# jinlinyi/PerspectiveFields

Hardware: NVIDIA H100
Metric: images/sec at 640x480 (Paramnet-360Cities-edina), H100 vs ref CPU (higher is better)
Workload: dtype f32 via 3x bf16 split MMA, fp32 accumulate

## Files before the change

### include/pf_b200.h

```cpp
#ifndef PF_B200_H_
#define PF_B200_H_

#include <stddef.h>
#include <stdint.h>

#ifdef __cplusplus
extern "C" {
#endif

#define PF_ABI_VERSION 3

typedef struct pf_engine* pf_handle;

enum pf_status { PF_OK = 0, PF_ERR_ARG = -1, PF_ERR_CUDA = -2, PF_ERR_WEIGHT = -3, PF_ERR_WORKSPACE = -4 };

enum pf_dtype { PF_F32 = 0, PF_BF16 = 1 };

enum pf_param_net { PF_PARAM_NONE = 0, PF_PARAM_CENTERED = 1 , PF_PARAM_UNCENTERED = 2  };

typedef struct pf_model_desc {
  int gravity_classes;
  int latitude_classes;
  int param_net;
  int param_input_size;
// ... 189 lines not shown
  int phase4;
  int npred; pf_tma_pred pred[2];
  int force_bn, force_kb;
  int picked_bn, picked_kb;
  int force_sched, picked_sched;
} pf_tma_op;
int pf_op_tma(pf_tma_op* op, void* stream);
int pf_op_tma_bf16(pf_tma_op* op, void* stream);
int pf_op_conv1_ring(const void* c_hi, const void* c_lo, int B, int H, int W, const float* wf, const float* bias, float* out,
                     const float* pg_w, const float* pg_b, float* pg_out, const float* pl_w, const float* pl_b, float* pl_out, void* stream);
int pf_tma_pick_tile(int mode, int64_t M, int N, int K, int sm_count, int* bn, int* kb);
int pf_op_pn_wgrad(const float* dy, int ldy, const float* x, const void* x_hi, const void* x_lo, int op, int ldx, int64_t R, int N, int K,
                   float* out, int* S, int* chunk, void* stream);
int pf_op_pn_colsum(const float* src, int64_t R, int C, float* out, void* stream);
int pf_op_pn_ln_bwd(const float* x, const float* dy, int64_t R, int C, const float* w, float* dx, float* g, void* stream);
int pf_op_pn_dw7_bwd(const float* x, const float* dt, int B, int H, int W, int C, const float* w_rot, float* dw, float* dx, int* rows_per_block,
                     void* stream);
int pf_op_pn_stem_bwd(const float* pin, const float* dS, const float* w, int B, int OH, int OW, float* dw, float* dpin, int* rows_per_block,
                      void* stream);
int pf_op_pn_fields_grad(const float* dpin, int B, int IH, int IW, int OH, int OW, float* dgrav, float* dlat, void* stream);
int pf_op_pn_tail_bwd(const float* feat, int n, int HW, const float* nw, const float* nb, const float* hw, const float* draw, float* dx,
                      float* grads, void* stream);
int pf_op_pn_pw2_grads(const float* G, const float* sdy, int C, int K, const float* gamma, const void* w_hi, const void* w_lo, const float* b,
                       float* dW, float* db, float* dgamma, void* stream);
int pf_op_pn_gelu_bwd(const float* dh, float* u, int64_t n, void* hi, void* lo, void* stream);
int pf_op_pn_scale_split(const float* src, const float* scale, int64_t n, int C, void* hi, void* lo, void* stream);
int pf_op_pn_col2im2(const float* dP, int B, int H, int W, int C, float* out, void* stream);
int pf_op_layernorm(const float* x, float* y, int64_t rows, int C, const float* w, const float* b, float eps, void* stream);
int pf_op_attention_tc(const float* q, const float* kv, float* out, int B, int N, int C, int heads, void* stream);
int pf_op_attention_tc_bf16(const float* q, const float* kv, float* out, int B, int N, int C, int heads, void* stream);
int pf_op_attention_tc_keys(const float* q, const float* kv, float* out, int B, int N, int NKV, int C, int heads, int bf16, void* stream);
int pf_op_dwconv3x3_gelu(const float* x, float* y, int B, int H, int W, int C, const float* w9c, const float* bias, void* stream);
int pf_op_dwconv7x7(const float* x, float* y, int B, int H, int W, int C, const float* w49c, const float* bias, void* stream);
int pf_op_upsample2x(const float* x, float* y, int B, int H, int W, int C, void* stream);
int pf_op_preprocess(const uint8_t* img_dev, int H, int W, const float* mean3, const float* std3, float* y, void* stream);
int pf_op_preprocess_sized(const uint8_t* img_dev, int H, int W, int net_h, int net_w, const float* mean3, const float* std3, float* y, void* stream);
int pf_op_resize_u8(const uint8_t* img_dev, int H, int W, int new_h, int new_w, uint8_t* out_dev, void* stream);
int pf_op_resize_f32(const float* img_dev, int H, int W, int C, int new_h, int new_w, float* out_dev, void* stream);
int pf_op_fill_stream(float* dst, int64_t numel, float value, void* stream);
int pf_op_argmax_decode(const float* logits, float* field, int B, int HW, int NC, int is_gravity, void* stream);
int pf_op_pred_argmax_decode(const float* feat, int ld, int coff, const float* w, const float* bias, float* field, int B, int HW, int NC,
                             int is_gravity, void* stream);
int pf_op_postprocess(const float* vec, const float* lat, int n, const int32_t* height, const int32_t* width,
                      float* gravity_original, const int64_t* gravity_original_offset, float* latitude_original,
                      const int64_t* latitude_original_offset, int lat_is_sin, void* stream);
int pf_op_postprocess_sized(const float* vec, const float* lat, int n, int net_h, int net_w, const int32_t* height, const int32_t* width,
                            float* gravity_original, const int64_t* gravity_original_offset, float* latitude_original,
                            const int64_t* latitude_original_offset, int lat_is_sin, void* stream);

#ifdef __cplusplus
}
#endif
#endif
```

### perspectivefields_b200/_native.py

```python
import ctypes
import os
import subprocess

_HERE = os.path.dirname(os.path.abspath(__file__))
ROOT = os.path.dirname(_HERE)
LIB_PATH = os.path.join(_HERE, "libpf_b200.so")
SRC_DIR = os.path.join(_HERE, "csrc")
HEADER = os.path.join(ROOT, "include", "pf_b200.h")

PF_F32, PF_BF16 = 0, 1
PF_PARAM_NONE, PF_PARAM_CENTERED, PF_PARAM_UNCENTERED = 0, 1, 2

NVCC_FLAGS = ["-gencode", "arch=compute_90a,code=sm_90a", "-O3", "-lineinfo", "-std=c++17",
              "-Xcompiler", "-fPIC", "-shared", "-ldl"]


class pf_model_desc(ctypes.Structure):
    _fields_ = [("gravity_classes", ctypes.c_int), ("latitude_classes", ctypes.c_int), ("param_net", ctypes.c_int),
                ("param_input_size", ctypes.c_int), ("pixel_mean", ctypes.c_float * 3), ("pixel_std", ctypes.c_float * 3)]


class pf_camera(ctypes.Structure):
    _fields_ = [("height", ctypes.c_int32), ("width", ctypes.c_int32), ("focal_rel", ctypes.c_double), ("elevation", ctypes.c_double),
                ("roll", ctypes.c_double), ("cx_rel", ctypes.c_double), ("cy_rel", ctypes.c_double),
# ... 149 lines not shown
        "pf_camera_fields": (i32, [i32, ctypes.POINTER(pf_camera), i32, vp, vp, vp]),
        "pf_camera_fields_vp": (i32, [i32, ctypes.POINTER(pf_camera), ctypes.POINTER(ctypes.c_double), i32, vp, vp, vp]),
        "pf_draw_fields": (i32, [i32, ctypes.POINTER(pf_draw_canvas), i32, vp, vp, vp, vp, vp]),
        "pf_pano_views": (i32, [i32, vp, i32, i32, ctypes.POINTER(pf_pano_view), i32, vp, vp, vp, vp, vp, vp, vp, vp, vp]),
        "pf_equi_views": (i32, [i32, vp, i32, i32, i32, i32, ctypes.POINTER(pf_equi_view), i32, i32, i32, i32, vp, vp]),
        "pf_encode_fields": (i32, [i32, i32, i32, i32, vp, ctypes.POINTER(i64), vp, ctypes.POINTER(i64), i32, i32, i32, vp, vp, vp]),
        "pf_head_losses_workspace": (i64, [i32, i32, i32, i32, i32]),
        "pf_head_losses": (i32, [i32, i32, i32, i32, i32, vp, vp, i32, vp, vp, i32, i32, f32, f32, vp, vp, i64, vp]),
        "pf_field_errors_workspace": (i64, [ctypes.POINTER(pf_field_image), i32, i32]),
        "pf_field_errors": (i32, [i32, ctypes.POINTER(pf_field_image), i32, vp, vp, vp, vp, vp, i32, ctypes.POINTER(ctypes.c_double), i32,
                                  vp, vp, vp, vp, vp, vp, vp, i64, vp]),
        "pf_fit_camera_workspace": (i64, [ctypes.POINTER(pf_fit_image), i32]),
        "pf_fit_camera": (i32, [i32, ctypes.POINTER(pf_fit_image), i32, vp, vp, vp, i32, ctypes.c_double, i32, vp, vp, vp, vp, vp, i64, vp]),
        "pf_rectify_workspace": (i64, [ctypes.POINTER(pf_rectify_image), i32]),
        "pf_rectify_views": (i32, [i32, ctypes.POINTER(pf_rectify_image), i32, vp, vp, vp, vp, i32, vp, i32, i32, ctypes.c_double, i32,
                                   ctypes.POINTER(ctypes.c_int32), vp, vp, vp, i64, vp]),
        "pf_op_pn_wgrad": (i32, [vp, i32, vp, vp, vp, i32, i32, i64, i32, i32, vp, ctypes.POINTER(i32), ctypes.POINTER(i32), vp]),
        "pf_op_pn_colsum": (i32, [vp, i64, i32, vp, vp]),
        "pf_op_pn_ln_bwd": (i32, [vp, vp, i64, i32, vp, vp, vp, vp]),
        "pf_op_pn_dw7_bwd": (i32, [vp, vp, i32, i32, i32, i32, vp, vp, vp, ctypes.POINTER(i32), vp]),
        "pf_op_pn_stem_bwd": (i32, [vp, vp, vp, i32, i32, i32, vp, vp, ctypes.POINTER(i32), vp]),
        "pf_op_pn_fields_grad": (i32, [vp, i32, i32, i32, i32, i32, vp, vp, vp]),
        "pf_op_pn_tail_bwd": (i32, [vp, i32, i32, vp, vp, vp, vp, vp, vp, vp]),
        "pf_op_pn_pw2_grads": (i32, [vp, vp, i32, i32, vp, vp, vp, vp, vp, vp, vp, vp]),
        "pf_op_pn_gelu_bwd": (i32, [vp, vp, i64, vp, vp, vp]),
        "pf_op_pn_scale_split": (i32, [vp, vp, i64, i32, vp, vp, vp]),
        "pf_op_pn_col2im2": (i32, [vp, i32, i32, i32, i32, vp, vp]),
        "pf_op_layernorm": (i32, [vp, vp, i64, i32, vp, vp, f32, vp]),
        "pf_op_attention_tc": (i32, [vp, vp, vp, i32, i32, i32, i32, vp]),
        "pf_op_attention_tc_bf16": (i32, [vp, vp, vp, i32, i32, i32, i32, vp]),
        "pf_op_attention_tc_keys": (i32, [vp, vp, vp, i32, i32, i32, i32, i32, i32, vp]),
        "pf_op_dwconv3x3_gelu": (i32, [vp, vp, i32, i32, i32, i32, vp, vp, vp]),
        "pf_op_dwconv7x7": (i32, [vp, vp, i32, i32, i32, i32, vp, vp, vp]),
        "pf_op_upsample2x": (i32, [vp, vp, i32, i32, i32, i32, vp]),
        "pf_op_preprocess": (i32, [vp, i32, i32, ctypes.POINTER(f32), ctypes.POINTER(f32), vp, vp]),
        "pf_op_preprocess_sized": (i32, [vp, i32, i32, i32, i32, ctypes.POINTER(f32), ctypes.POINTER(f32), vp, vp]),
        "pf_op_resize_u8": (i32, [vp, i32, i32, i32, i32, vp, vp]),
        "pf_op_resize_f32": (i32, [vp, i32, i32, i32, i32, i32, vp, vp]),
        "pf_op_argmax_decode": (i32, [vp, vp, i32, i32, i32, i32, vp]),
        "pf_op_fill_stream": (i32, [vp, i64, f32, vp]),
        "pf_op_pred_argmax_decode": (i32, [vp, i32, i32, vp, vp, vp, i32, i32, i32, i32, vp]),
        "pf_op_postprocess": (i32, [vp, vp, i32, ctypes.POINTER(ctypes.c_int32), ctypes.POINTER(ctypes.c_int32), vp, ctypes.POINTER(i64), vp,
                                    ctypes.POINTER(i64), i32, vp]),
        "pf_op_postprocess_sized": (i32, [vp, vp, i32, i32, i32, ctypes.POINTER(ctypes.c_int32), ctypes.POINTER(ctypes.c_int32), vp,
                                          ctypes.POINTER(i64), vp, ctypes.POINTER(i64), i32, vp]),
        "pf_comm_unique_id": (i32, [vp]),
        "pf_comm_create": (i32, [i32, i32, i32, vp, ctypes.POINTER(vp)]),
        "pf_comm_destroy": (i32, [vp]),
        "pf_gather": (i32, [vp, i32, i32, ctypes.POINTER(vp), ctypes.POINTER(i64), ctypes.POINTER(ctypes.c_int32), vp]),
        "pf_jpeg_create": (i32, [i32, i32, ctypes.POINTER(vp)]),
        "pf_jpeg_destroy": (i32, [vp]),
        "pf_jpeg_info": (i32, [vp, vp, i64, ctypes.POINTER(ctypes.c_int32), ctypes.POINTER(ctypes.c_int32)]),
        "pf_jpeg_decode_batch": (i32, [vp, i32, ctypes.POINTER(vp), ctypes.POINTER(i64), ctypes.POINTER(ctypes.c_int32),
                                       ctypes.POINTER(ctypes.c_int32), vp, ctypes.POINTER(i64), vp]),
    }
    for name, (res, args) in sig.items():
        try:
            fn = getattr(L, name)
        except AttributeError:
            if os.environ.get("PF_B200_LIB"):
                continue
            raise
        fn.restype, fn.argtypes = res, args
    if L.pf_abi_version() != 3:
        raise RuntimeError("libpf_b200.so ABI version mismatch")
    _lib = L
    return L


EXPORTS = ["pf_abi_version", "pf_last_error", "pf_kernel_launch_count", "pf_create", "pf_create_sized", "pf_destroy", "pf_set_weight",
           "pf_finalize", "pf_workspace_bytes", "pf_forward", "pf_param_workspace_bytes", "pf_param_forward", "pf_param_train_workspace_bytes",
           "pf_param_train_forward", "pf_param_backward", "pf_param_grad_numel", "pf_param_grad_entry", "pf_profile_enable", "pf_profile_read", "pf_profile_kernels_enable",
           "pf_profile_kernels_read", "pf_set_option", "pf_debug_enable", "pf_debug_count", "pf_debug_name", "pf_debug_numel",
           "pf_debug_copy", "pf_camera_fields", "pf_camera_fields_vp", "pf_pano_views", "pf_equi_views", "pf_draw_fields",
           "pf_encode_fields", "pf_head_losses_workspace", "pf_head_losses", "pf_field_errors_workspace", "pf_field_errors",
           "pf_fit_camera_workspace", "pf_fit_camera", "pf_rectify_workspace", "pf_rectify_views", "pf_comm_unique_id", "pf_comm_create", "pf_comm_destroy", "pf_gather",
           "pf_jpeg_create", "pf_jpeg_destroy", "pf_jpeg_info", "pf_jpeg_decode_batch",
           "pf_op_conv_gemm", "pf_op_tma", "pf_op_tma_bf16", "pf_op_conv1_ring", "pf_tma_pick_tile", "pf_op_layernorm",
           "pf_op_attention_tc", "pf_op_attention_tc_bf16", "pf_op_attention_tc_keys", "pf_op_dwconv3x3_gelu",
           "pf_op_dwconv7x7", "pf_op_upsample2x", "pf_op_preprocess", "pf_op_preprocess_sized", "pf_op_fill_stream", "pf_op_resize_u8",
           "pf_op_resize_f32", "pf_op_argmax_decode", "pf_op_pred_argmax_decode", "pf_op_postprocess", "pf_op_postprocess_sized",
           "pf_op_pn_wgrad", "pf_op_pn_colsum", "pf_op_pn_ln_bwd", "pf_op_pn_dw7_bwd", "pf_op_pn_stem_bwd", "pf_op_pn_fields_grad",
           "pf_op_pn_tail_bwd", "pf_op_pn_pw2_grads", "pf_op_pn_gelu_bwd", "pf_op_pn_scale_split", "pf_op_pn_col2im2"]


class PfError(RuntimeError):
    pass


def check(status):
    if status < 0:
        raise PfError(f"libpf_b200: {lib().pf_last_error().decode()} (status {status})")
    return status
```

### perspectivefields_b200/csrc/layers.cuh

```cuda
#pragma once
#include "common.cuh"

namespace pf {

template <int KH, int KW, int STRIDE, int PAD, int COUT, int PPT, int PGROUPS>
__global__ void __launch_bounds__(COUT* PGROUPS) stem_conv_kernel(const float* __restrict__ in, int ldin, int B, int H, int W,
                                                                  const float* __restrict__ w, const float* __restrict__ bias,
                                                                  float* __restrict__ out, int OH, int OW) {
  constexpr int PIX = PPT * PGROUPS;
  constexpr int IN_W = (PIX - 1) * STRIDE + KW;
  __shared__ float s_in[KH][IN_W][3];
  const int tiles_x = cdiv(OW, PIX);
  int bid = blockIdx.x;
  const int tx = bid % tiles_x; bid /= tiles_x;
  const int oy = bid % OH; const int b = bid / OH;
  const int ox0 = tx * PIX;
  const int iy0 = oy * STRIDE - PAD, ix0 = ox0 * STRIDE - PAD;
  for (int i = threadIdx.x; i < KH * IN_W * 3; i += blockDim.x) {
    const int c = i % 3, x = (i / 3) % IN_W, y = i / (3 * IN_W);
    const int iy = iy0 + y, ix = ix0 + x;
    float v = 0.f;
    if ((unsigned)iy < (unsigned)H && (unsigned)ix < (unsigned)W) v = __ldg(in + ((long long)(b * H + iy) * W + ix) * ldin + c);
    s_in[y][x][c] = v;
  }
// ... 219 lines not shown
            acc[oy][p].z = fmaf(a[p + kx].z, kk.z, acc[oy][p].z); acc[oy][p].w = fmaf(a[p + kx].w, kk.w, acc[oy][p].w);
          }
        }
      }
    }
#endif
#pragma unroll
    for (int oy = 0; oy < 2; ++oy) {
      if (y0 + oy >= H) break;
#pragma unroll
      for (int p = 0; p < PX; ++p) {
        if (!cv[p + 1]) break;
        const float4 o = make_float4(gelu_erf(acc[oy][p].x), gelu_erf(acc[oy][p].y), gelu_erf(acc[oy][p].z), gelu_erf(acc[oy][p].w));
        const unsigned oi = o00 + (unsigned)oy * rs + (unsigned)p * C4;
        if (out) reinterpret_cast<float4*>(out)[oi] = o;
        if (shi) {
          uint2 h, l;
          split_bf16x2(o.x, o.y, h.x, l.x);
          split_bf16x2(o.z, o.w, h.y, l.y);
          reinterpret_cast<uint2*>(shi)[oi] = h;
          reinterpret_cast<uint2*>(slo)[oi] = l;
        }
      }
    }
  }
}

#ifndef PF_DW7_PX
#define PF_DW7_PX 4
#endif
#ifndef PF_DW7_MINBLOCKS
#define PF_DW7_MINBLOCKS 2
#endif
__global__ void __launch_bounds__(256, PF_DW7_MINBLOCKS) dwconv7x7_kernel(const float* __restrict__ in, float* __restrict__ out, int B, int H, int W, int C,
                                                        const float* __restrict__ w, const float* __restrict__ bias) {
  pdl_wait();
  pdl_launch();
  constexpr int PX = PF_DW7_PX;
  const unsigned C4 = (unsigned)C >> 2, XG = ((unsigned)W + PX - 1) / PX, YG = ((unsigned)H + 1) >> 1;
  const unsigned total = (unsigned)B * YG * XG * C4;
  const unsigned rs = (unsigned)W * C4;
  const float4* __restrict__ in4 = reinterpret_cast<const float4*>(in);
  const float4* __restrict__ w4 = reinterpret_cast<const float4*>(w);
  for (unsigned i = blockIdx.x * blockDim.x + threadIdx.x; i < total; i += gridDim.x * blockDim.x) {
    const unsigned c4 = i % C4;
    unsigned r = i / C4;
    const unsigned xg = r % XG; r /= XG;
    const int y0 = (int)(r % YG) * 2; const unsigned b = r / YG;
    const int x0 = (int)xg * PX;
    const unsigned o00 = ((b * (unsigned)H + (unsigned)y0) * (unsigned)W + (unsigned)x0) * C4 + c4;
    bool cv[PX + 6];
#pragma unroll
    for (int j = 0; j < PX + 6; ++j) cv[j] = (unsigned)(x0 - 3 + j) < (unsigned)W;
    const float4 bv = __ldg(reinterpret_cast<const float4*>(bias) + c4);
    float4 acc[2][PX];
#pragma unroll
    for (int oy = 0; oy < 2; ++oy)
#pragma unroll
      for (int p = 0; p < PX; ++p) acc[oy][p] = bv;
#pragma unroll
    for (int ry = 0; ry < 8; ++ry) {
      const int iy = y0 + ry - 3;
      if ((unsigned)iy >= (unsigned)H) continue;
      const unsigned rb = o00 + (unsigned)(ry - 3) * rs - 3u * C4;
      float4 a[PX + 6];
#pragma unroll
      for (int j = 0; j < PX + 6; ++j) {
        a[j] = make_float4(0.f, 0.f, 0.f, 0.f);
        if (cv[j]) a[j] = __ldg(in4 + (rb + (unsigned)j * C4));
      }
#pragma unroll
      for (int oy = 0; oy < 2; ++oy) {
        const int ky = ry - oy;
        if (ky < 0 || ky > 6) continue;
#pragma unroll
        for (int kx = 0; kx < 7; ++kx) {
          const float4 k = __ldg(w4 + ((unsigned)(ky * 7 + kx) * C4 + c4));
#pragma unroll
          for (int p = 0; p < PX; ++p) {
            acc[oy][p].x = fmaf(a[p + kx].x, k.x, acc[oy][p].x); acc[oy][p].y = fmaf(a[p + kx].y, k.y, acc[oy][p].y);
            acc[oy][p].z = fmaf(a[p + kx].z, k.z, acc[oy][p].z); acc[oy][p].w = fmaf(a[p + kx].w, k.w, acc[oy][p].w);
          }
        }
      }
    }
#pragma unroll
    for (int oy = 0; oy < 2; ++oy) {
      if (y0 + oy >= H) break;
#pragma unroll
      for (int p = 0; p < PX; ++p) {
        if (!cv[p + 3]) break;
        reinterpret_cast<float4*>(out)[o00 + (unsigned)oy * rs + (unsigned)p * C4] = acc[oy][p];
      }
    }
  }
}

inline unsigned ew_grid(long long total) {
  long long g = cdivl(total, 256);
  const long long cap = 132LL * 32;
  return (unsigned)(g < cap ? (g > 0 ? g : 1) : cap);
}

inline long long upsample2x_threads(int B, int H, int W, int C) { return (long long)B * H * ((W + 1) / 2) * (C / 4); }
__global__ void __launch_bounds__(256) upsample2x_kernel(const float* __restrict__ in, int ldi, int icoff, float* __restrict__ out, int ldo, int ocoff,
                                                         int B, int H, int W, int C, __nv_bfloat16* __restrict__ shi = nullptr, __nv_bfloat16* __restrict__ slo = nullptr) {
  pdl_wait();
  pdl_launch();
  const unsigned C4 = (unsigned)C >> 2, JG = ((unsigned)W + 1) >> 1, li4 = (unsigned)ldi >> 2, lo4 = (unsigned)ldo >> 2;
  const unsigned total = (unsigned)B * H * JG * C4;
  const unsigned OW = 2u * W;
  const float4* __restrict__ in4 = reinterpret_cast<const float4*>(in + icoff);
  const unsigned oc4 = (unsigned)ocoff >> 2;
  for (unsigned i = blockIdx.x * blockDim.x + threadIdx.x; i < total; i += gridDim.x * blockDim.x) {
    const unsigned c4 = i % C4;
    unsigned r = i / C4;
    const unsigned jg = r % JG; r /= JG;
    const int iy = (int)(r % (unsigned)H); const unsigned b = r / (unsigned)H;
    const int j0 = (int)jg * 2;
    const bool two = j0 + 1 < W;
    const int cx[4] = {j0 > 0 ? j0 - 1 : 0, j0, j0 + 1 < W ? j0 + 1 : W - 1, j0 + 2 < W ? j0 + 2 : W - 1};
    const int cy[3] = {iy > 0 ? iy - 1 : 0, iy, iy + 1 < H ? iy + 1 : H - 1};
    float4 t[3][4];
#pragma unroll
    for (int ry = 0; ry < 3; ++ry) {
      const unsigned rb = ((b * (unsigned)H + (unsigned)cy[ry]) * (unsigned)W) * li4 + c4;
      float4 v[4];
#pragma unroll
// ... 399 lines not shown
```

### perspectivefields_b200/csrc/pf_b200.cu

```cuda
#include "../../include/pf_b200.h"

#include <cuda_runtime.h>
#include <nvtx3/nvToolsExt.h>

#include <atomic>
#include <cctype>
#include <cmath>
#include <cstdarg>
#include <cstdio>
#include <cstdlib>
#include <cstring>
#include <map>
#include <mutex>
#include <string>
#include <functional>
#include <unordered_map>
#include <vector>

#include "common.cuh"
#include "tma_host.cuh"
#include "attention_mma.cuh"
#include "layers.cuh"
#include "prepost.cuh"
#include "pano.cuh"
// ... 422 lines not shown
    } else { maps.a2_hi = maps.a_hi; maps.a2_lo = maps.a_lo; }
    if (!msg) msg = map2d(&maps.b_hi, w.hi, p.K, (long long)groups * N, p.K, bn, kb);
    if (!msg) msg = map2d(&maps.b_lo, w.lo, p.K, (long long)groups * N, p.K, bn, kb);
    if (msg) return fail(PF_ERR_CUDA, "%s", msg);
    return launch_tma(MODE_HALO, maps, p, bn, kb, pp, pred);
  }
  int tconv_gather(const SplitT& A, int B, int H, int W, int Cin, int KH, int stride, int pad, const GemmW& w, int N, const Epi& o) {
    const int OH = (H + 2 * pad - KH) / stride + 1, OW = (W + 2 * pad - KH) / stride + 1;
    const long long M = (long long)B * OH * OW;
    const int K = KH * KH * Cin;
    const long long m = ar.mark();
    SplitT col = salloc(M, K);
    if (!dry) {
      if (Cin % 8) return fail(PF_ERR_ARG, "tconv_gather: Cin %% 8");
      LAUNCHED(launch_pdl(im2col_split_kernel, dim3(ew_grid(M * K / 8)), dim3(256), 0, st, A.hi, A.lo, A.ld, col.hi, col.lo, B, H, W, Cin, OH, OW, KH, stride, pad));
    }
    int r = tgemm(col, M, K, 0, w, N, o);
    ar.release(m);
    return r;
  }
  int ln_split(const float* x, const SplitT& y, long long rows, int C, const LnW& w, float eps, float* yf = nullptr) {
    if (dry) return PF_OK;
    LAUNCHED(layernorm_launch(x, yf, rows, C, w.w, w.b, eps, st, y));
    return PF_OK;
  }
  int ln_split_patch(const float* x, const SplitT& y, const SplitT& patch, long long rows, int C, const LnW& w, float eps, int RH, int RW, int sr) {
    if (dry) return PF_OK;
    LAUNCHED(layernorm_launch(x, nullptr, rows, C, w.w, w.b, eps, st, y, patch, RH, RW, sr));
    return PF_OK;
  }
  int ln(const float* x, float* y, long long rows, int C, const LnW& w, float eps) {
    if (dry) return PF_OK;
    LAUNCHED(layernorm_launch(x, y, rows, C, w.w, w.b, eps, st));
    return PF_OK;
  }
};

constexpr long long kTableSlabBytes = 8LL << 20;
static int get_table(pf_engine* e, int in_size, int out_size, pf_engine::DevTable* out, cudaStream_t st) {
  auto it = e->tables.find({in_size, out_size});
  if (it == e->tables.end()) {
    ResampleTable t = make_resample_table(in_size, out_size);
    const long long nb = (long long)t.bounds.size() * sizeof(int), nc = (long long)t.coeffs.size() * sizeof(int);
    const long long need = ((nb + 255) & ~255LL) + ((nc + 255) & ~255LL);
    if (need > kTableSlabBytes) return fail(PF_ERR_ARG, "image axis of %d pixels is too long for the resize tables", in_size);
    if (e->table_off + need > kTableSlabBytes) {
      CU(cudaStreamSynchronize(st));
      e->tables.clear();
      e->table_off = 0;
    }
    pf_engine::DevTable d{};
    d.ksize = t.ksize;
    const long long o0 = e->table_off, o1 = o0 + ((nb + 255) & ~255LL);
    memcpy(e->table_host + o0, t.bounds.data(), nb);
    memcpy(e->table_host + o1, t.coeffs.data(), nc);
    d.bounds = (int*)(e->table_dev + o0);
    d.coeffs = (int*)(e->table_dev + o1);
    CU(cudaMemcpyAsync(e->table_dev + o0, e->table_host + o0, need, cudaMemcpyHostToDevice, st));
    e->table_off += need;
    it = e->tables.emplace(std::make_pair(in_size, out_size), d).first;
  }
  *out = it->second;
  return PF_OK;
}

static int pre_rows_needed(int H, int OH) {
// ... 303 lines not shown

static int fwd_paramnet(Fwd& F, const float* grav, const float* lat, float* params, float* raw, const PnSaved* sv) {
  pf_engine* e = F.e;
  const pf_model_desc& D = e->desc;
  const int n = F.n;
  const bool dry = F.dry;
  cudaStream_t st = F.st;
  Arena& ar = F.ar;
  using Epi = Fwd::Epi;
  const int NH = e->net_h, NW = e->net_w;
  {
    if (D.gravity_classes != 2 || D.latitude_classes != 1) return fail(PF_ERR_ARG, "ParamNet needs regression heads");
    const bool centered = D.param_net == PF_PARAM_CENTERED;
    const int SH = centered ? NH : D.param_input_size, SW = centered ? NW : D.param_input_size;
    float* pin = sv ? sv->pin : ar.f((long long)n * SH * SW * 4);
    if (!dry) LAUNCHED((pack_fields_kernel<<<(unsigned)cdivl((long long)n * SH * SW, 256), 256, 0, st>>>(grav, lat, pin, n, NH, NW, SH, SW), cudaGetLastError()));
    int rh = SH / 4, rw = SW / 4;
    float* x = sv ? sv->xs[0][0] : ar.f((long long)n * rh * rw * 96);
    float* stem = sv ? sv->stem_pre : x;
    if (!dry) LAUNCHED((stem_conv_launch<4, 4, 4, 0, 96>(pin, 4, n, SH, SW, e->pn_stem_w, e->pn_stem_b, stem, st)));
    TRY(F.ln(stem, x, (long long)n * rh * rw, 96, e->pn_stem_ln, 1e-6f));
    for (int s = 0; s < 4; ++s) {
      const int C = kCnxDims[s];
      if (s > 0) {
        const int r2h = rh / 2, r2w = rw / 2;
        SplitT y = F.salloc((long long)n * r2h * r2w, 4 * kCnxDims[s - 1]);
        TRY(F.ln_split_patch(x, SplitT(), y, (long long)n * rh * rw, kCnxDims[s - 1], e->pn_ds_ln[s], 1e-6f, rh, rw, 2));
        float* xn = sv ? sv->xs[s][0] : ar.f((long long)n * r2h * r2w * C);
        Epi o; o.C = xn; o.ldc = C;
        TRY(F.tgemm(y, (long long)n * r2h * r2w, 4 * kCnxDims[s - 1], 0, e->pn_ds[s], C, o));
        x = xn; rh = r2h; rw = r2w;
      }
      const long long rows = (long long)n * rh * rw;
      float* yf = ar.f(rows * C);
      SplitT y = F.salloc(rows, C);
      SplitT h = F.salloc(rows, 4 * C);
      for (int j = 0; j < kCnxDepths[s]; ++j) {
        const CnxBlockW& b = e->pn_blocks[s][j];
        if (!dry) LAUNCHED(launch_pdl(dwconv7x7_kernel, dim3(ew_grid((long long)n * ((rh + 1) / 2) * ((rw + PF_DW7_PX - 1) / PF_DW7_PX) * (C / 4))), dim3(256), 0, st, x, yf, n, rh, rw, C, b.dw_w, b.dw_b));
        TRY(F.ln_split(yf, y, rows, C, b.ln, 1e-6f));
        { Epi o; o.S = h; o.act = 2; TRY(F.tgemm(y, rows, C, 0, b.pw1, 4 * C, o)); }
        float* xo = sv ? sv->xs[s][j + 1] : x;
        { Epi o; o.C = xo; o.ldc = C; o.res = x; o.ldr = C; o.gamma = b.gamma; TRY(F.tgemm(h, rows, 4 * C, 0, b.pw2, C, o)); }
        x = xo;
      }
      TRY(F.tapf(x, rows * C, "cnx.s%d", s));
    }
    if (!dry) {
      if (!params) return fail(PF_ERR_ARG, "params output is NULL");
      LAUNCHED((param_tail_kernel<<<n, 256, 0, st>>>(x, rh * rw, e->pn_norm.w, e->pn_norm.b, e->pn_head_w, e->pn_head_b, params, raw, D.param_net), cudaGetLastError()));
    }
  }
  return PF_OK;
}

static void pn_input_size(const pf_engine* e, int* SH, int* SW) {
  const bool centered = e->desc.param_net == PF_PARAM_CENTERED;
  *SH = centered ? e->net_h : e->desc.param_input_size;
  *SW = centered ? e->net_w : e->desc.param_input_size;
}

static void pn_saved_alloc(Fwd& F, PnSaved& sv) {
  int SH, SW;
  pn_input_size(F.e, &SH, &SW);
  const long long n = F.n;
  sv.pin = F.ar.f(n * SH * SW * 4);
  int rh = SH / 4, rw = SW / 4;
  sv.stem_pre = F.ar.f(n * rh * rw * 96);
  for (int s = 0; s < 4; ++s) {
    if (s > 0) { rh /= 2; rw /= 2; }
    for (int j = 0; j <= kCnxDepths[s]; ++j) sv.xs[s][j] = F.ar.f(n * rh * rw * kCnxDims[s]);
  }
}
// ... 167 lines not shown
}

static int pn_pw2_grads(Fwd& F, const float* G, const float* sdy, int C, int K, const float* gamma, const GemmW& w2, float* dW, float* db, float* dgamma) {
  if (!F.dry) LAUNCHED((pw2_grads_kernel<<<cdiv(C, 8), 256, 0, F.st>>>(G, sdy, C, K, gamma, w2.hi, w2.lo, w2.b, dW, db, dgamma), cudaGetLastError()));
  return PF_OK;
}
static int pn_gelu_bwd(Fwd& F, const float* dh, float* u, long long n, __nv_bfloat16* hi, __nv_bfloat16* lo) {
  if (!F.dry) LAUNCHED((gelu_bwd_kernel<<<ew_grid(n), 256, 0, F.st>>>(dh, u, n, hi, lo), cudaGetLastError()));
  return PF_OK;
}
static int pn_scale_split(Fwd& F, const float* src, const float* scale, long long n, int C, const SplitT& out) {
  if (!F.dry) LAUNCHED((scale_split_kernel<<<ew_grid(n), 256, 0, F.st>>>(src, scale, n, C, out.hi, out.lo), cudaGetLastError()));
  return PF_OK;
}
static int pn_col2im2(Fwd& F, const float* dP, int rh, int rw, int C, float* out) {
  if (!F.dry) LAUNCHED((col2im2_kernel<<<ew_grid((long long)F.n * rh * rw * C), 256, 0, F.st>>>(dP, F.n, rh, rw, C, out), cudaGetLastError()));
  return PF_OK;
}

static int pn_block_bwd(Fwd& F, int s, int j, const float* xin, float* dx, int rh, int rw, float* grads) {
  pf_engine* e = F.e;
  Arena& ar = F.ar;
  const bool dry = F.dry;
  cudaStream_t st = F.st;
  const int C = kCnxDims[s];
  const long long R = (long long)F.n * rh * rw;
  const CnxBlockW& b = e->pn_blocks[s][j];
  const auto& T = e->pn_train;
  char nm[64];
  snprintf(nm, sizeof nm, "pn.s%d.b%d.", s, j);
  const std::string P(nm);
  const long long m0 = ar.mark();
  float* t = ar.f(R * C);
  TRY(pn_dw_launch(F, xin, t, rh, rw, C, b.dw_w, b.dw_b));
  SplitT ys = F.salloc(R, C);
  TRY(F.ln_split(t, ys, R, C, b.ln, 1e-6f));
  float* u = ar.f(R * 4 * C);
  { Fwd::Epi o; o.C = u; o.ldc = 4 * C; TRY(F.tgemm(ys, R, C, 0, b.pw1, 4 * C, o)); }
  {
    const long long m1 = ar.mark();
    float* G = ar.f(4LL * C * C);
    float* sdx = ar.f(C);
    TRY(pn_wgrad_full(F, dx, C, nullptr, u, 1, 4 * C, R, C, 4 * C, G));
    TRY(pn_colsum(F, dx, R, C, sdx));
    TRY(pn_pw2_grads(F, G, sdx, C, 4 * C, b.gamma, b.pw2, grads + pn_goff(P + "pw2.w"), grads + pn_goff(P + "pw2.b"), grads + pn_goff(P + "gamma")));
    ar.release(m1);
  }
  {
    const long long m1 = ar.mark();
    SplitT dz = F.salloc(R, C);
    TRY(pn_scale_split(F, dx, b.gamma, R * C, C, dz));
    float* dh = ar.f(R * 4 * C);
    { Fwd::Epi o; o.C = dh; o.ldc = 4 * C; TRY(F.tgemm(dz, R, C, 0, T.pw2_t[s][j], 4 * C, o)); }
    TRY(pn_gelu_bwd(F, dh, u, R * 4 * C, nullptr, nullptr));
    ar.release(m1);
  }
  TRY(pn_wgrad_full(F, u, 4 * C, &ys, nullptr, 0, C, R, 4 * C, C, grads + pn_goff(P + "pw1.w")));
  TRY(pn_colsum(F, u, R, 4 * C, grads + pn_goff(P + "pw1.b")));
  float* dy = ar.f(R * C);
  {
    const long long m1 = ar.mark();
    SplitT du = F.salloc(R, 4 * C);
    TRY(pn_scale_split(F, u, nullptr, R * 4 * C, 4 * C, du));
    Fwd::Epi o; o.C = dy; o.ldc = C;
    TRY(F.tgemm(du, R, 4 * C, 0, T.pw1_t[s][j], C, o));
    ar.release(m1);
  }
  float* dt = ar.f(R * C);
  TRY(pn_ln_bwd(F, t, dy, R, C, b.ln.w, dt, grads + pn_goff(P + "ln.w")));
// ... 1471 lines not shown
  if (le != cudaSuccess) r = fail(PF_ERR_CUDA, "split_kernel: %s", cudaGetErrorString(le));
  if (r == PF_OK) {
    le = attention_mma_launch(nullptr, B, N, C, heads, st, as, qs, kvs, np, nkv);
    if (le != cudaSuccess) r = fail(PF_ERR_CUDA, "attention_mma_launch: %s", cudaGetErrorString(le));
  }
  if (r == PF_OK) {
    le = (merge_split_kernel<<<(unsigned)cdivl(nq, 256), 256, 0, st>>>(as.hi, as.lo, out, nq), cudaGetLastError());
    if (le != cudaSuccess) r = fail(PF_ERR_CUDA, "merge_split_kernel: %s", cudaGetErrorString(le));
  }
  cudaError_t se = cudaStreamSynchronize(st);
  cudaFree(scratch);
  if (r == PF_OK && se != cudaSuccess) r = fail(PF_ERR_CUDA, "pf_op_attention_tc: %s", cudaGetErrorString(se));
  return r;
}
int pf_op_attention_tc(const float* q, const float* kv, float* out, int B, int N, int C, int heads, void* stream) {
  return op_attention_tc(q, kv, out, B, N, C, heads, stream, 3);
}
int pf_op_attention_tc_bf16(const float* q, const float* kv, float* out, int B, int N, int C, int heads, void* stream) {
  return op_attention_tc(q, kv, out, B, N, C, heads, stream, 1);
}
int pf_op_attention_tc_keys(const float* q, const float* kv, float* out, int B, int N, int NKV, int C, int heads, int bf16, void* stream) {
  return op_attention_tc(q, kv, out, B, N, C, heads, stream, bf16 ? 1 : 3, NKV);
}
int pf_op_dwconv3x3_gelu(const float* x, float* y, int B, int H, int W, int C, const float* w, const float* bias, void* stream) {
  if (C % 4) return fail(PF_ERR_ARG, "C %% 4");
  LAUNCHED(launch_pdl(dwconv3x3_gelu_kernel, dim3(ew_grid((long long)B * ((H + 1) / 2) * ((W + PF_DW3_PX - 1) / PF_DW3_PX) * (C / 4))), dim3(256), 0, (cudaStream_t)stream, x, y, B, H, W, C, w, bias, nullptr, nullptr));
  return PF_OK;
}
int pf_op_dwconv7x7(const float* x, float* y, int B, int H, int W, int C, const float* w, const float* bias, void* stream) {
  if (C % 4) return fail(PF_ERR_ARG, "C %% 4");
  LAUNCHED(launch_pdl(dwconv7x7_kernel, dim3(ew_grid((long long)B * ((H + 1) / 2) * ((W + PF_DW7_PX - 1) / PF_DW7_PX) * (C / 4))), dim3(256), 0, (cudaStream_t)stream, x, y, B, H, W, C, w, bias));
  return PF_OK;
}
int pf_op_upsample2x(const float* x, float* y, int B, int H, int W, int C, void* stream) {
  if (C % 4) return fail(PF_ERR_ARG, "C %% 4");
  LAUNCHED(launch_pdl(upsample2x_kernel, dim3(ew_grid(upsample2x_threads(B, H, W, C))), dim3(256), 0, (cudaStream_t)stream, x, C, 0, y, C, 0, B, H, W, C, nullptr, nullptr));
  return PF_OK;
}
int pf_op_preprocess(const uint8_t* img, int H, int W, const float* mean3, const float* std3, float* y, void* stream) {
  return pf_op_preprocess_sized(img, H, W, kNet, kNet, mean3, std3, y, stream);
}
int pf_op_preprocess_sized(const uint8_t* img, int H, int W, int net_h, int net_w, const float* mean3, const float* std3, float* y, void* stream) {
  if (!img || !mean3 || !std3 || !y || H < 1 || W < 1) return fail(PF_ERR_ARG, "pf_op_preprocess: bad argument");
  if (!net_size_ok(net_h, net_w)) return fail(PF_ERR_ARG, "pf_op_preprocess: unsupported working size %dx%d", net_h, net_w);
  TRY(configure_current_device());
  ResampleTable tx = make_resample_table(W, net_w), ty = make_resample_table(H, net_h);
  const int max_rows = pre_max_smem_rows(net_w);
  if (ty.ksize + 1 > max_rows) return fail(PF_ERR_ARG, "image too tall");
  int *bx, *cx, *by, *cy;
  PreImage* d;
  CU(cudaMalloc(&bx, tx.bounds.size() * 4)); CU(cudaMalloc(&cx, tx.coeffs.size() * 4));
  CU(cudaMalloc(&by, ty.bounds.size() * 4)); CU(cudaMalloc(&cy, ty.coeffs.size() * 4));
  CU(cudaMalloc(&d, sizeof(PreImage)));
  CU(cudaMemcpy(bx, tx.bounds.data(), tx.bounds.size() * 4, cudaMemcpyHostToDevice));
  CU(cudaMemcpy(cx, tx.coeffs.data(), tx.coeffs.size() * 4, cudaMemcpyHostToDevice));
  CU(cudaMemcpy(by, ty.bounds.data(), ty.bounds.size() * 4, cudaMemcpyHostToDevice));
  CU(cudaMemcpy(cy, ty.coeffs.data(), ty.coeffs.size() * 4, cudaMemcpyHostToDevice));
  PreImage pi{0, H, W, tx.ksize, ty.ksize, bx, cx, by, cy};
  CU(cudaMemcpy(d, &pi, sizeof pi, cudaMemcpyHostToDevice));
  int rows = pre_rows_needed(H, net_h);
  if (rows > max_rows) rows = max_rows;
  const int smem = rows * net_w * 3;
  LAUNCHED((preprocess_kernel<<<dim3(net_h / kPreRows, 1), net_w, smem, (cudaStream_t)stream>>>(img, d, y, mean3[0], mean3[1], mean3[2], std3[0], std3[1], std3[2], rows,
                                                                                                 net_h, net_w),
            cudaGetLastError()));
  CU(cudaStreamSynchronize((cudaStream_t)stream));
// ... 6 lines not shown
```

Baseline: 809.1.

## Fuse depthwise 7x7 conv with LayerNorm and bf16 split in ParamNet blocks

Adds a kernel that runs the depthwise 7x7 convolution, stages the output tile in shared memory, then applies LayerNorm and writes the hi/lo bf16 split directly. The ConvNeXt block forward path (and the backward recompute) now use it instead of a separate dwconv kernel plus ln_split, which removes the fp32 intermediate write and re-read plus one launch. The trade-off is per-block shared memory and thread counts that depend on C, which may lower occupancy. Support is restricted to 64 < C <= 768.

```diff
diff --git a/include/pf_b200.h b/include/pf_b200.h
--- a/include/pf_b200.h
+++ b/include/pf_b200.h
@@ -245,6 +245,8 @@
 int pf_op_attention_tc_keys(const float* q, const float* kv, float* out, int B, int N, int NKV, int C, int heads, int bf16, void* stream);
 int pf_op_dwconv3x3_gelu(const float* x, float* y, int B, int H, int W, int C, const float* w9c, const float* bias, void* stream);
 int pf_op_dwconv7x7(const float* x, float* y, int B, int H, int W, int C, const float* w49c, const float* bias, void* stream);
+int pf_op_dwconv7x7_ln(const float* x, float* y, void* hi, void* lo, int B, int H, int W, int C, const float* w49c, const float* bias,
+                       const float* ln_w, const float* ln_b, float eps, void* stream);
 int pf_op_upsample2x(const float* x, float* y, int B, int H, int W, int C, void* stream);
 int pf_op_preprocess(const uint8_t* img_dev, int H, int W, const float* mean3, const float* std3, float* y, void* stream);
 int pf_op_preprocess_sized(const uint8_t* img_dev, int H, int W, int net_h, int net_w, const float* mean3, const float* std3, float* y, void* stream);
diff --git a/perspectivefields_b200/_native.py b/perspectivefields_b200/_native.py
--- a/perspectivefields_b200/_native.py
+++ b/perspectivefields_b200/_native.py
@@ -205,6 +205,7 @@
         "pf_op_attention_tc_keys": (i32, [vp, vp, vp, i32, i32, i32, i32, i32, i32, vp]),
         "pf_op_dwconv3x3_gelu": (i32, [vp, vp, i32, i32, i32, i32, vp, vp, vp]),
         "pf_op_dwconv7x7": (i32, [vp, vp, i32, i32, i32, i32, vp, vp, vp]),
+        "pf_op_dwconv7x7_ln": (i32, [vp, vp, vp, vp, i32, i32, i32, i32, vp, vp, vp, vp, f32, vp]),
         "pf_op_upsample2x": (i32, [vp, vp, i32, i32, i32, i32, vp]),
         "pf_op_preprocess": (i32, [vp, i32, i32, ctypes.POINTER(f32), ctypes.POINTER(f32), vp, vp]),
         "pf_op_preprocess_sized": (i32, [vp, i32, i32, i32, i32, ctypes.POINTER(f32), ctypes.POINTER(f32), vp, vp]),
@@ -251,7 +252,7 @@
            "pf_jpeg_create", "pf_jpeg_destroy", "pf_jpeg_info", "pf_jpeg_decode_batch",
            "pf_op_conv_gemm", "pf_op_tma", "pf_op_tma_bf16", "pf_op_conv1_ring", "pf_tma_pick_tile", "pf_op_layernorm",
            "pf_op_attention_tc", "pf_op_attention_tc_bf16", "pf_op_attention_tc_keys", "pf_op_dwconv3x3_gelu",
-           "pf_op_dwconv7x7", "pf_op_upsample2x", "pf_op_preprocess", "pf_op_preprocess_sized", "pf_op_fill_stream", "pf_op_resize_u8",
+           "pf_op_dwconv7x7", "pf_op_dwconv7x7_ln", "pf_op_upsample2x", "pf_op_preprocess", "pf_op_preprocess_sized", "pf_op_fill_stream", "pf_op_resize_u8",
            "pf_op_resize_f32", "pf_op_argmax_decode", "pf_op_pred_argmax_decode", "pf_op_postprocess", "pf_op_postprocess_sized",
            "pf_op_pn_wgrad", "pf_op_pn_colsum", "pf_op_pn_ln_bwd", "pf_op_pn_dw7_bwd", "pf_op_pn_stem_bwd", "pf_op_pn_fields_grad",
            "pf_op_pn_tail_bwd", "pf_op_pn_pw2_grads", "pf_op_pn_gelu_bwd", "pf_op_pn_scale_split", "pf_op_pn_col2im2"]
diff --git a/perspectivefields_b200/csrc/layers.cuh b/perspectivefields_b200/csrc/layers.cuh
--- a/perspectivefields_b200/csrc/layers.cuh
+++ b/perspectivefields_b200/csrc/layers.cuh
@@ -275,6 +275,43 @@
 #ifndef PF_DW7_MINBLOCKS
 #define PF_DW7_MINBLOCKS 2
 #endif
+template <int PX>
+__device__ __forceinline__ void dw7_tile(const float4* __restrict__ in4, const float4* __restrict__ w4, const float* __restrict__ bias,
+                                         int H, unsigned C4, unsigned rs, unsigned o00, unsigned c4, int y0, const bool (&cv)[PX + 6],
+                                         float4 (&acc)[2][PX]) {
+  const float4 bv = __ldg(reinterpret_cast<const float4*>(bias) + c4);
+#pragma unroll
+  for (int oy = 0; oy < 2; ++oy)
+#pragma unroll
+    for (int p = 0; p < PX; ++p) acc[oy][p] = bv;
+#pragma unroll
+  for (int ry = 0; ry < 8; ++ry) {
+    const int iy = y0 + ry - 3;
+    if ((unsigned)iy >= (unsigned)H) continue;
+    const unsigned rb = o00 + (unsigned)(ry - 3) * rs - 3u * C4;
+    float4 a[PX + 6];
+#pragma unroll
+    for (int j = 0; j < PX + 6; ++j) {
+      a[j] = make_float4(0.f, 0.f, 0.f, 0.f);
+      if (cv[j]) a[j] = __ldg(in4 + (rb + (unsigned)j * C4));
+    }
+#pragma unroll
+    for (int oy = 0; oy < 2; ++oy) {
+      const int ky = ry - oy;
+      if (ky < 0 || ky > 6) continue;
+#pragma unroll
+      for (int kx = 0; kx < 7; ++kx) {
+        const float4 k = __ldg(w4 + ((unsigned)(ky * 7 + kx) * C4 + c4));
+#pragma unroll
+        for (int p = 0; p < PX; ++p) {
+          acc[oy][p].x = fmaf(a[p + kx].x, k.x, acc[oy][p].x); acc[oy][p].y = fmaf(a[p + kx].y, k.y, acc[oy][p].y);
+          acc[oy][p].z = fmaf(a[p + kx].z, k.z, acc[oy][p].z); acc[oy][p].w = fmaf(a[p + kx].w, k.w, acc[oy][p].w);
+        }
+      }
+    }
+  }
+}
+
 __global__ void __launch_bounds__(256, PF_DW7_MINBLOCKS) dwconv7x7_kernel(const float* __restrict__ in, float* __restrict__ out, int B, int H, int W, int C,
                                                         const float* __restrict__ w, const float* __restrict__ bias) {
   pdl_wait();
@@ -295,38 +332,8 @@
     bool cv[PX + 6];
 #pragma unroll
     for (int j = 0; j < PX + 6; ++j) cv[j] = (unsigned)(x0 - 3 + j) < (unsigned)W;
-    const float4 bv = __ldg(reinterpret_cast<const float4*>(bias) + c4);
     float4 acc[2][PX];
-#pragma unroll
-    for (int oy = 0; oy < 2; ++oy)
-#pragma unroll
-      for (int p = 0; p < PX; ++p) acc[oy][p] = bv;
-#pragma unroll
-    for (int ry = 0; ry < 8; ++ry) {
-      const int iy = y0 + ry - 3;
-      if ((unsigned)iy >= (unsigned)H) continue;
-      const unsigned rb = o00 + (unsigned)(ry - 3) * rs - 3u * C4;
-      float4 a[PX + 6];
-#pragma unroll
-      for (int j = 0; j < PX + 6; ++j) {
-        a[j] = make_float4(0.f, 0.f, 0.f, 0.f);
-        if (cv[j]) a[j] = __ldg(in4 + (rb + (unsigned)j * C4));
-      }
-#pragma unroll
-      for (int oy = 0; oy < 2; ++oy) {
-        const int ky = ry - oy;
-        if (ky < 0 || ky > 6) continue;
-#pragma unroll
-        for (int kx = 0; kx < 7; ++kx) {
-          const float4 k = __ldg(w4 + ((unsigned)(ky * 7 + kx) * C4 + c4));
-#pragma unroll
-          for (int p = 0; p < PX; ++p) {
-            acc[oy][p].x = fmaf(a[p + kx].x, k.x, acc[oy][p].x); acc[oy][p].y = fmaf(a[p + kx].y, k.y, acc[oy][p].y);
-            acc[oy][p].z = fmaf(a[p + kx].z, k.z, acc[oy][p].z); acc[oy][p].w = fmaf(a[p + kx].w, k.w, acc[oy][p].w);
-          }
-        }
-      }
-    }
+    dw7_tile<PX>(in4, w4, bias, H, C4, rs, o00, c4, y0, cv, acc);
 #pragma unroll
     for (int oy = 0; oy < 2; ++oy) {
       if (y0 + oy >= H) break;
@@ -337,6 +344,133 @@
       }
     }
   }
+}
+
+#ifndef PF_DW7LN_TILE_THREADS
+#define PF_DW7LN_TILE_THREADS 128
+#endif
+constexpr int kDw7LnMaxThreads = 256;
+__host__ __device__ __forceinline__ unsigned dw7_ln_tiles(unsigned C4) {
+  return C4 < PF_DW7LN_TILE_THREADS ? PF_DW7LN_TILE_THREADS / C4 : 1u;
+}
+template <int MAXQ>
+__global__ void __launch_bounds__(kDw7LnMaxThreads, PF_DW7_MINBLOCKS)
+    dwconv7x7_ln_kernel(const float* __restrict__ in, float* __restrict__ yf, int B, int H, int W, int C, const float* __restrict__ w,
+                        const float* __restrict__ bias, const float* __restrict__ gw, const float* __restrict__ gb, float eps,
+                        __nv_bfloat16* __restrict__ shi, __nv_bfloat16* __restrict__ slo) {
+  pdl_wait();
+  pdl_launch();
+  constexpr int PX = PF_DW7_PX, TP = 2 * PX;
+  extern __shared__ float4 s_y[];
+  const unsigned C4 = (unsigned)C >> 2, XG = ((unsigned)W + PX - 1) / PX, YG = ((unsigned)H + 1) >> 1;
+  const unsigned T = dw7_ln_tiles(C4), tiles = (unsigned)B * YG * XG;
+  const unsigned rs = (unsigned)W * C4;
+  const float4* __restrict__ in4 = reinterpret_cast<const float4*>(in);
+  {
+    const unsigned t = threadIdx.x / C4, c4 = threadIdx.x % C4, tile = blockIdx.x * T + t;
+    if (t < T && tile < tiles) {
+      const unsigned xg = tile % XG, r = tile / XG;
+      const int y0 = (int)(r % YG) * 2; const unsigned b = r / YG;
+      const int x0 = (int)xg * PX;
+      const unsigned o00 = ((b * (unsigned)H + (unsigned)y0) * (unsigned)W + (unsigned)x0) * C4 + c4;
+      bool cv[PX + 6];
+#pragma unroll
+      for (int j = 0; j < PX + 6; ++j) cv[j] = (unsigned)(x0 - 3 + j) < (unsigned)W;
+      float4 acc[2][PX];
+      dw7_tile<PX>(in4, reinterpret_cast<const float4*>(w), bias, H, C4, rs, o00, c4, y0, cv, acc);
+#pragma unroll
+      for (int oy = 0; oy < 2; ++oy)
+#pragma unroll
+        for (int p = 0; p < PX; ++p) {
+          s_y[(t * TP + oy * PX + p) * C4 + c4] = acc[oy][p];
+          if (yf && y0 + oy < H && cv[p + 3]) reinterpret_cast<float4*>(yf)[o00 + (unsigned)oy * rs + (unsigned)p * C4] = acc[oy][p];
+        }
+    }
+  }
+  __syncthreads();
+  constexpr int NR = 2;
+  const unsigned lane = threadIdx.x & 31, Q = C4, nw = blockDim.x >> 5;
+  const float inv_c = 1.0f / (float)C;
+  float4 wq[MAXQ], bq[MAXQ];
+#pragma unroll
+  for (int i = 0; i < MAXQ; ++i) {
+    const unsigned qd = lane + 32 * i;
+    if (qd < Q) { wq[i] = __ldg(reinterpret_cast<const float4*>(gw) + qd); bq[i] = __ldg(reinterpret_cast<const float4*>(gb) + qd); }
+  }
+  for (unsigned k0 = threadIdx.x >> 5; k0 < T * TP; k0 += NR * nw) {
+    float4 v[NR][MAXQ];
+    float s[NR], q[NR];
+    unsigned ob[NR];
+    bool ok[NR];
+#pragma unroll
+    for (int j = 0; j < NR; ++j) {
+      const unsigned k = k0 + j * nw, tile = blockIdx.x * T + k / TP;
+      const unsigned xg = tile % XG, r = tile / XG;
+      const unsigned y = (r % YG) * 2 + (k % TP) / PX, b = r / YG, x = xg * PX + k % PX;
+      ok[j] = k < T * TP && tile < tiles && y < (unsigned)H && x < (unsigned)W;
+      ob[j] = ((b * (unsigned)H + y) * (unsigned)W + x) * Q;
+      s[j] = 0.f;
+#pragma unroll
+      for (int i = 0; i < MAXQ; ++i) {
+        const unsigned qd = lane + 32 * i;
+        v[j][i] = make_float4(0.f, 0.f, 0.f, 0.f);
+        if (ok[j] && qd < Q) v[j][i] = s_y[k * C4 + qd];
+        s[j] += (v[j][i].x + v[j][i].y) + (v[j][i].z + v[j][i].w);
+      }
+    }
+#pragma unroll
+    for (int o = 16; o > 0; o >>= 1)
+#pragma unroll
+      for (int j = 0; j < NR; ++j) s[j] += __shfl_xor_sync(0xffffffffu, s[j], o);
+#pragma unroll
+    for (int j = 0; j < NR; ++j) {
+      s[j] *= inv_c;
+      q[j] = 0.f;
+#pragma unroll
+      for (int i = 0; i < MAXQ; ++i) {
+        if (lane + 32 * i < Q) {
+          const float a = v[j][i].x - s[j], bb = v[j][i].y - s[j], c = v[j][i].z - s[j], d = v[j][i].w - s[j];
+          q[j] = fmaf(a, a, q[j]); q[j] = fmaf(bb, bb, q[j]); q[j] = fmaf(c, c, q[j]); q[j] = fmaf(d, d, q[j]);
+        }
+      }
+    }
+#pragma unroll
+    for (int o = 16; o > 0; o >>= 1)
+#pragma unroll
+      for (int j = 0; j < NR; ++j) q[j] += __shfl_xor_sync(0xffffffffu, q[j], o);
+#pragma unroll
+    for (int j = 0; j < NR; ++j) {
+      if (!ok[j]) continue;
+      const float mean = s[j];
+      const float rstd = 1.0f / sqrtf(fmaf(q[j], inv_c, eps));
+#pragma unroll
+      for (int i = 0; i < MAXQ; ++i) {
+        const unsigned qd = lane + 32 * i;
+        if (qd < Q) {
+          const float4 o = make_float4((v[j][i].x - mean) * rstd * wq[i].x + bq[i].x, (v[j][i].y - mean) * rstd * wq[i].y + bq[i].y,
+                                       (v[j][i].z - mean) * rstd * wq[i].z + bq[i].z, (v[j][i].w - mean) * rstd * wq[i].w + bq[i].w);
+          uint2 h, l;
+          split_bf16x2(o.x, o.y, h.x, l.x);
+          split_bf16x2(o.z, o.w, h.y, l.y);
+          reinterpret_cast<uint2*>(shi)[ob[j] + qd] = h;
+          reinterpret_cast<uint2*>(slo)[ob[j] + qd] = l;
+        }
+      }
+    }
+  }
+}
+
+inline cudaError_t dwconv7x7_ln_launch(const float* in, float* yf, int B, int H, int W, int C, const float* w, const float* bias,
+                                       const float* gw, const float* gb, float eps, SplitT y, cudaStream_t st) {
+  if (C <= 64 || C > 768 || C % 4 || y.ld != C || !y.hi || !y.lo || B < 1 || H < 1 || W < 1 || (long long)B * H * W * (C / 4) >= (1LL << 31))
+    return cudaErrorInvalidValue;
+  const int C4 = C / 4, T = (int)dw7_ln_tiles((unsigned)C4);
+  const long long tiles = (long long)B * ((H + 1) / 2) * ((W + PF_DW7_PX - 1) / PF_DW7_PX);
+  const dim3 grid((unsigned)cdivl(tiles, T)), block((unsigned)cdiv(T * C4, 32) * 32);
+  const size_t smem = (size_t)T * 2 * PF_DW7_PX * C4 * sizeof(float4);
+  if (C <= 128) return launch_pdl(dwconv7x7_ln_kernel<1>, grid, block, smem, st, in, yf, B, H, W, C, w, bias, gw, gb, eps, y.hi, y.lo);
+  if (C <= 384) return launch_pdl(dwconv7x7_ln_kernel<3>, grid, block, smem, st, in, yf, B, H, W, C, w, bias, gw, gb, eps, y.hi, y.lo);
+  return launch_pdl(dwconv7x7_ln_kernel<6>, grid, block, smem, st, in, yf, B, H, W, C, w, bias, gw, gb, eps, y.hi, y.lo);
 }
 
 inline unsigned ew_grid(long long total) {
diff --git a/perspectivefields_b200/csrc/pf_b200.cu b/perspectivefields_b200/csrc/pf_b200.cu
--- a/perspectivefields_b200/csrc/pf_b200.cu
+++ b/perspectivefields_b200/csrc/pf_b200.cu
@@ -478,6 +478,11 @@
   int ln(const float* x, float* y, long long rows, int C, const LnW& w, float eps) {
     if (dry) return PF_OK;
     LAUNCHED(layernorm_launch(x, y, rows, C, w.w, w.b, eps, st));
+    return PF_OK;
+  }
+  int dw7_ln(const float* x, float* yf, const SplitT& y, int rh, int rw, int C, const CnxBlockW& b) {
+    if (dry) return PF_OK;
+    LAUNCHED(dwconv7x7_ln_launch(x, yf, n, rh, rw, C, b.dw_w, b.dw_b, b.ln.w, b.ln.b, 1e-6f, y, st));
     return PF_OK;
   }
 };
@@ -847,13 +852,11 @@
         x = xn; rh = r2h; rw = r2w;
       }
       const long long rows = (long long)n * rh * rw;
-      float* yf = ar.f(rows * C);
       SplitT y = F.salloc(rows, C);
       SplitT h = F.salloc(rows, 4 * C);
       for (int j = 0; j < kCnxDepths[s]; ++j) {
         const CnxBlockW& b = e->pn_blocks[s][j];
-        if (!dry) LAUNCHED(launch_pdl(dwconv7x7_kernel, dim3(ew_grid((long long)n * ((rh + 1) / 2) * ((rw + PF_DW7_PX - 1) / PF_DW7_PX) * (C / 4))), dim3(256), 0, st, x, yf, n, rh, rw, C, b.dw_w, b.dw_b));
-        TRY(F.ln_split(yf, y, rows, C, b.ln, 1e-6f));
+        TRY(F.dw7_ln(x, nullptr, y, rh, rw, C, b));
         { Epi o; o.S = h; o.act = 2; TRY(F.tgemm(y, rows, C, 0, b.pw1, 4 * C, o)); }
         float* xo = sv ? sv->xs[s][j + 1] : x;
         { Epi o; o.C = xo; o.ldc = C; o.res = x; o.ldr = C; o.gamma = b.gamma; TRY(F.tgemm(h, rows, 4 * C, 0, b.pw2, C, o)); }
@@ -1087,9 +1090,8 @@
   const std::string P(nm);
   const long long m0 = ar.mark();
   float* t = ar.f(R * C);
-  TRY(pn_dw_launch(F, xin, t, rh, rw, C, b.dw_w, b.dw_b));
   SplitT ys = F.salloc(R, C);
-  TRY(F.ln_split(t, ys, R, C, b.ln, 1e-6f));
+  TRY(F.dw7_ln(xin, t, ys, rh, rw, C, b));
   float* u = ar.f(R * 4 * C);
   { Fwd::Epi o; o.C = u; o.ldc = 4 * C; TRY(F.tgemm(ys, R, C, 0, b.pw1, 4 * C, o)); }
   {
@@ -2627,6 +2629,13 @@
   LAUNCHED(launch_pdl(dwconv7x7_kernel, dim3(ew_grid((long long)B * ((H + 1) / 2) * ((W + PF_DW7_PX - 1) / PF_DW7_PX) * (C / 4))), dim3(256), 0, (cudaStream_t)stream, x, y, B, H, W, C, w, bias));
   return PF_OK;
 }
+int pf_op_dwconv7x7_ln(const float* x, float* y, void* hi, void* lo, int B, int H, int W, int C, const float* w, const float* bias,
+                       const float* ln_w, const float* ln_b, float eps, void* stream) {
+  if (!x || !hi || !lo || !w || !bias || !ln_w || !ln_b) return fail(PF_ERR_ARG, "pf_op_dwconv7x7_ln: NULL argument");
+  const SplitT ys{(__nv_bfloat16*)hi, (__nv_bfloat16*)lo, C};
+  LAUNCHED(dwconv7x7_ln_launch(x, y, B, H, W, C, w, bias, ln_w, ln_b, eps, ys, (cudaStream_t)stream));
+  return PF_OK;
+}
 int pf_op_upsample2x(const float* x, float* y, int B, int H, int W, int C, void* stream) {
   if (C % 4) return fail(PF_ERR_ARG, "C %% 4");
   LAUNCHED(launch_pdl(upsample2x_kernel, dim3(ew_grid(upsample2x_threads(B, H, W, C))), dim3(256), 0, (cudaStream_t)stream, x, C, 0, y, C, 0, B, H, W, C, nullptr, nullptr));
```

New measurement: 808.5 (median of 6 runs). Within noise of the previous version (-0.1%).
